# ccaven/tinyslam

Hardware: AMD Instinct MI355X
Metric: ORB extract throughput, 1280x720 (frames/sec; Mkeypoints/sec alongside) (higher is better)
Workload: dtype f32; 1 GPU; BASELINE.json configs[3]: batch of 256 independent 1280x720 RGBA frames per GPU, device-resident, full ORB (FAST-12 + orientation + blur + BRIEF-256); frames_per_gpu_per_batch=256, width=1280, height=720, hierarchy_depth=2, max_features=8192, content=default, mode=literal, input=rgba, pipeline=default, fp_contract=0, angle_bins=0, batches_in_flight=1, collate=none (1 GPU)

## Files before the change

### include/tinyorb.h

```cpp
#ifndef TINYORB_H
#define TINYORB_H

#include <stddef.h>
#include <stdint.h>

#ifdef __cplusplus
extern "C" {
#endif

#define TINYORB_ABI_VERSION 5

#define ORB_OK 0
#define ORB_EINVAL 1
#define ORB_EHIP 2
#define ORB_ECAPACITY 3
#define ORB_ESTATE 4

#define ORB_MAX_HIERARCHY_DEPTH 10

typedef struct OrbExtent3d {
    uint32_t width;
    uint32_t height;
    uint32_t depth_or_array_layers;
} OrbExtent3d;
// ... 260 lines not shown
#define ORB_TRACK_MATCHED 2u

typedef struct {
    uint32_t prev;
    uint32_t next;
    uint32_t head_index;
    uint16_t head_frame;
    uint16_t tail_frame;
} OrbTrack;

typedef struct {
    uint32_t keypoints;
    uint32_t links_in;
    uint32_t links_out;
    uint32_t keyframe;
    uint32_t ref_keyframe;
    uint32_t shared;
    uint32_t reserved[2];
} OrbTrackFrame;

int orb_track_consecutive(OrbProgram *p, uint32_t n_frames, const OrbTrackParams *params, void *stream);
int orb_track_read(OrbProgram *p, uint32_t frame, OrbTrack *dst, size_t n);
int orb_track_frames(OrbProgram *p, OrbTrackFrame *dst, size_t n);

void orb_corner_level0_xy(const CornerData *c, float *x0, float *y0);

#define ORB_PLANE_GRAY 0
#define ORB_PLANE_BLUR 1
int orb_debug_read_plane(OrbProgram *p, uint32_t frame, int kind, uint32_t level, uint16_t *dst, size_t n_texels);
int orb_level_size(const OrbProgram *p, uint32_t level, uint32_t *width, uint32_t *height);
int orb_debug_f32_to_f16(OrbProgram *p, const float *src, uint16_t *dst, size_t n);
int orb_debug_angle_code(OrbProgram *p, const float *cy, const float *cx, uint32_t *dst, size_t n);
int orb_debug_rot_table(OrbProgram *p, int16_t *dst, size_t n_entries, uint32_t *codes, uint32_t *pitch);
int orb_debug_pose_buffers(OrbProgram *p, void **matches, void **poses, void **points);

#define ORB_KERNEL_COUNT 25
int orb_profile_enable(OrbProgram *p, int enable);
int orb_profile_reset(OrbProgram *p);
int orb_profile_get(OrbProgram *p, int id, double *total_ms, uint64_t *launches);
const char *orb_kernel_name(int id);

#define ORB_SYN_GRADIENT 1u
#define ORB_SYN_BLOBS 2u
#define ORB_SYN_WEDGES 4u
#define ORB_SYN_NOISE 8u
#define ORB_SYN_Y8 16u
int orb_synth_frames_device(OrbProgram *p, uint8_t *frames_dev, uint32_t n_frames, uint32_t seed0, uint32_t flags,
                            uint8_t **out_dev);
int orb_debug_stamps(OrbProgram *p, unsigned long long *dst, size_t n);
int orb_copy_to_host(OrbProgram *p, void *dst_host, const void *src_dev, size_t nbytes);

#ifdef __cplusplus
}
#endif
#endif
```

### tinyslam_amd/csrc/orb_api.hip

```cpp
#include <hip/hip_runtime.h>
#include <chrono>
#include <cmath>

#include <cstdarg>
#include <cstdio>
#include <cstdlib>
#include <cstring>
#include <new>
#include <optional>
#include <string>
#include <algorithm>
#include <vector>

#include "../../include/tinyorb.h"
#include "orb_front_launch.h"
#include "orb_kernels_fused.h"
#include "orb_kernels_brief.h"
#include "orb_kernels_intended.h"
#include "orb_kernels_staged.h"
#include "orb_kernels_collate.h"
#include "orb_kernels_match.h"
#include "orb_kernels_verify.h"
#include "orb_kernels_epipolar.h"
#include "orb_kernels_guide.h"
// ... 155 lines not shown
        bool no_swizzle = false, quiet = false;
        bool front_generic = false, front_trace = false;
        int phase_mask = -1, brief_i_mask = -1, lds_pad = 0;
    } env;
    uint32_t* dv_count = nullptr;
    CornerData* dv_corners = nullptr;
    CornerDescriptor* dv_desc = nullptr;
    uint16_t* d_gray = nullptr;
    uint16_t* d_blur = nullptr;
    uint16_t* d_blur_rowc = nullptr;
    uint32_t blur_qa[kMaxLevels] = {0};
    uint32_t* d_counts = nullptr;
    CornerData* d_corners = nullptr;
    CornerDescriptor* d_desc = nullptr;
    uint32_t* out_counts[2] = {nullptr, nullptr};
    CornerData* out_corners[2] = {nullptr, nullptr};
    CornerDescriptor* out_desc[2] = {nullptr, nullptr};
    CornerData* d_seg = nullptr;
    uint32_t* d_seg_counts = nullptr;
    uint32_t* d_seg_before = nullptr;
    uint64_t* d_nf_mask[2] = {nullptr, nullptr};
    BandGeom bands{};
    RowsGeom rows{};
    BriefTGeom brieft{};
    bool use_brief_t = false;
    uint32_t band_rows_lvl[kMaxLevels] = {0};
    uint32_t ln_threads[kMaxLevels] = {0};
    uint32_t tile_w_lvl[kMaxLevels] = {0};
    uint32_t seg_classes = 1;
    uint32_t* d_pattern = nullptr;
    float* d_cos = nullptr;
    float* d_sin = nullptr;
    uint4* d_rot = nullptr;
    unsigned long long* d_stamps = nullptr;

    uint32_t* h_count = nullptr;
    uint32_t* d_single_done = nullptr;
    hipEvent_t single_done_ev = nullptr;
    uint32_t single_seq = 0;
    CornerData* h_corners = nullptr;
    CornerDescriptor* h_desc = nullptr;
    bool single_valid = false;

    uint32_t last_batch = 0;
    hipStream_t last_stream = nullptr;
    bool planes_valid = false;
    bool fused = false;
    uint32_t max_lds = 0;
    uint32_t n_cus = 256;

    bool profiling = false;
    std::vector<ProfSpan> pending;
    std::vector<hipEvent_t> event_pool;
    double prof_ms[ORB_KERNEL_COUNT] = {0};
    uint64_t prof_n[ORB_KERNEL_COUNT] = {0};

    std::string pipeline_note;
    std::string err;
};

namespace {

int fail(OrbProgram* p, int code, const char* fmt, ...) {
    char buf[512];
    va_list ap;
    va_start(ap, fmt);
// ... 367 lines not shown
    for (uint32_t m = 0; m < p->pyr.depth; m++) {
        g.flat_end[m] = rg.flat_end[m];
        g.qa[m] = rg.qa[m];
        g.row_base[m] = rows + (uint32_t)kBriefHalo;
        rows += p->pyr.h[m] + 2u * (uint32_t)kBriefHalo + 8u;
    }
    g.rows_padded = rows;
    g.oob = p->oob;
    *out = g;
    if (getenv("TINYORB_BRIEF_ROWS")) return false;
    return rg.n_slots >= 1u && rg.n_slots * n_classes <= kBriefTMaxSlots && rows <= kBriefTMaxRows;
}

int launch_brief(OrbProgram* p, hipStream_t s, uint32_t n, const RowsGeom& rows_geom, const uint16_t* d_blur,
                 const uint16_t* d_blur_rowc, const uint32_t* seg_counts, uint32_t* seg_before, const CornerData* seg,
                 uint32_t* d_counts, CornerData* d_corners, CornerDescriptor* d_desc, uint32_t f0 = 0) {
    const uint32_t cap = p->cfg.max_features;
    const BriefTables tab{p->d_pattern, p->d_cos, p->d_sin, p->d_rot};
    const bool use_t = p->use_brief_t;
    {
        LaunchScope ls(p, s, KID_PREFIX);
        hipLaunchKernelGGL(k_slot_prefix, dim3(n), dim3(64), 0, s, seg_counts, seg_before, d_counts, rows_geom.n_slots,
                           rows_geom.seg_cap, use_t ? p->brieft.n_classes : 1u);
    }
    if (use_t) {
        const BriefTGeom& tg = p->brieft;
        const dim3 grid(n, (cap + (uint32_t)kBriefNfChunk - 1u) / (uint32_t)kBriefNfChunk);
        const uint32_t mask_words = brief_mask_words(cap);
        uint64_t* const nf_mask = p->d_nf_mask[p->cur_set] + (size_t)f0 * mask_words;
        {
            LaunchScope ls(p, s, KID_BRIEF_T);
#define BRIEF_T_LAUNCH(ROT_)                                                                                                         \
    hipLaunchKernelGGL((k_brief_t<kBriefTWaves, ROT_>), dim3(n, (cap + kBriefTThreads - 1u) / kBriefTThreads), dim3(kBriefTThreads), \
                       brieft_lds_bytes(tg), s, d_blur_rowc, p->pyr, tg, seg_counts, seg_before, seg, d_corners, cap, d_desc, tab, nf_mask, mask_words)
            switch (rot_form(p->opt.fp_contract)) {
                case 1: BRIEF_T_LAUNCH(1); break;
                case 2: BRIEF_T_LAUNCH(2); break;
                default: BRIEF_T_LAUNCH(0); break;
            }
#undef BRIEF_T_LAUNCH
        }
        LaunchScope ls(p, s, KID_BRIEF_NF);
#define BRIEF_NF_LAUNCH(OOB_, TABLE_)                                                                                                  \
    hipLaunchKernelGGL((k_brief_nf<OOB_, TABLE_>), grid, dim3(256), 0, s, d_blur, d_blur_rowc, p->pyr, tg, d_corners, cap, d_desc, tab, \
                       nf_mask, mask_words)
        const bool table = p->pyr.depth > 2u;
        if (p->oob != kOobZero) {
            if (table) BRIEF_NF_LAUNCH(true, true); else BRIEF_NF_LAUNCH(true, false);
        } else {
            if (table) BRIEF_NF_LAUNCH(false, true); else BRIEF_NF_LAUNCH(false, false);
        }
#undef BRIEF_NF_LAUNCH
    } else {
        LaunchScope ls(p, s, KID_BRIEF_ROWS);
        RowsGeom rg = rows_geom;
        rg.oob = p->oob;
        rg.fp = p->opt.fp_contract;
        rg.split = 1u;
        while (rg.split < 16u && rg.n_slots * n * rg.split < 2048u) rg.split *= 2u;
        hipLaunchKernelGGL(k_brief_rows, dim3(rg.n_slots * rg.split, n), dim3(256), 0, s, d_blur, d_blur_rowc, p->pyr, rg,
                           seg_counts, seg_before, seg, d_corners, cap, d_desc, tab);
    }
    return ORB_OK;
}

FrontGeom fused_level_geometry(const OrbProgram* p, uint32_t lvl, uint32_t gw, uint32_t gh, uint32_t n) {
    const Pyramid& pyr = p->pyr;
// ... 662 lines not shown
        for (uint32_t m = 0; m < p->pyr.depth; m++) {
            const uint32_t gw = ((width + 7u) / 8u) * 8u, gh = ((height + 7u) / 8u) * 8u;
            p->score_layout.off[m] = off;
            p->score_layout.pitch[m] = gw + 2u;
            off += (gw + 2u) * (gh + 2u);
            width /= 2u;
            height /= 2u;
        }
        p->score_layout.stride = (off + 63u) & ~63u;
        p->cap_prov = (uint32_t)std::min<uint64_t>(std::max<uint64_t>(p->pyr.stride, cap), 1u << 24);
        if (p->opt.flags & ORB_FLAG_NMS)
        CREATE_TRY(hipMalloc(&p->d_score_planes, B * (size_t)p->score_layout.stride * sizeof(float)));
        CREATE_TRY(hipMalloc(&p->d_prov_counts, B * sizeof(uint32_t)));
        CREATE_TRY(hipMalloc(&p->d_prov, B * (size_t)p->cap_prov * sizeof(CornerData)));
        CREATE_TRY(hipMalloc(&p->d_prov_scores, B * (size_t)p->cap_prov * sizeof(float)));
        if (p->intended && (p->opt.flags & ORB_FLAG_NMS)) {
            CREATE_TRY(hipMalloc(&p->d_prov2_counts, B * sizeof(uint32_t)));
            CREATE_TRY(hipMalloc(&p->d_prov2, B * (size_t)p->cap_prov * sizeof(CornerData)));
            CREATE_TRY(hipMalloc(&p->d_prov2_scores, B * (size_t)p->cap_prov * sizeof(float)));
        }
    }
    CREATE_TRY(hipMalloc(&p->d_pattern, 256 * sizeof(uint32_t)));
    CREATE_TRY(hipMalloc(&p->d_cos, ORB_ANGLE_STEPS_FULL * sizeof(float)));
    CREATE_TRY(hipMalloc(&p->d_sin, ORB_ANGLE_STEPS_FULL * sizeof(float)));
    CREATE_TRY(hipMemcpy(p->d_pattern, ORB_BRIEF_PATTERN, 1024, hipMemcpyHostToDevice));
    CREATE_TRY(hipMemcpy(p->d_cos, ORB_COS_BITS, ORB_ANGLE_STEPS_FULL * 4, hipMemcpyHostToDevice));
    CREATE_TRY(hipMemcpy(p->d_sin, ORB_SIN_BITS, ORB_ANGLE_STEPS_FULL * 4, hipMemcpyHostToDevice));
    {
        const uint32_t n_codes = p->fused_i ? (p->opt.angle_bins ? p->opt.angle_bins : (uint32_t)ORB_ANGLE_STEPS_FULL) : (uint32_t)ORB_ANGLE_STEPS;
        const int pitch = p->fused_i ? (int)p->itiles.pitch : kNfPatchCols;
        CREATE_TRY(hipMalloc(&p->d_rot, (size_t)n_codes * 64u * sizeof(uint4)));
        hipLaunchKernelGGL(k_rot_table, dim3(n_codes), dim3(64), 0, p->stream, p->d_pattern, p->d_cos, p->d_sin, pitch, p->fused_i ? 1 : 0, p->d_rot,
                           p->opt.fp_contract, p->fused_i ? p->opt.angle_bins : 0u);
        CREATE_TRY(hipGetLastError());
        CREATE_TRY(hipStreamSynchronize(p->stream));
    }
    if (p->fused && getenv("TINYORB_STAMPS")) {
        CREATE_TRY(hipMalloc(&p->d_stamps, 32 * sizeof(unsigned long long)));
        CREATE_TRY(hipMemset(p->d_stamps, 0, 32 * sizeof(unsigned long long)));
    }
    CREATE_TRY(hipHostMalloc(&p->h_count, kSingleCountWords * sizeof(uint32_t), hipHostMallocDefault));
    memset(p->h_count, 0, kSingleCountWords * sizeof(uint32_t));
    CREATE_TRY(hipMalloc(&p->d_single_done, sizeof(uint32_t)));
    CREATE_TRY(hipMemset(p->d_single_done, 0, sizeof(uint32_t)));
    CREATE_TRY(hipHostMalloc(&p->h_corners, cap * sizeof(CornerData), hipHostMallocDefault));
    CREATE_TRY(hipHostMalloc(&p->h_desc, cap * sizeof(CornerDescriptor), hipHostMallocDefault));
    {
        void *dc = nullptr, *dk = nullptr, *dd = nullptr;
        if (hipHostGetDevicePointer(&dc, p->h_count, 0) == hipSuccess && hipHostGetDevicePointer(&dk, p->h_corners, 0) == hipSuccess &&
            hipHostGetDevicePointer(&dd, p->h_desc, 0) == hipSuccess) {
            p->dv_count = static_cast<uint32_t*>(dc);
            p->dv_corners = static_cast<CornerData*>(dk);
            p->dv_desc = static_cast<CornerDescriptor*>(dd);
        } else {
            (void)hipGetLastError();
        }
    }
#undef CREATE_TRY
    *out = p;
    return ORB_OK;
}

void orb_program_destroy(OrbProgram* p) {
    if (!p) return;
    (void)hipSetDevice(p->device);
    if (p->stream) (void)hipStreamSynchronize(p->stream);
// ... 5 lines not shown
    (void)hipFree(p->d_input);
    (void)hipFree(p->d_input_alt);
    for (hipEvent_t ev : p->in_uploaded)
        if (ev) (void)hipEventDestroy(ev);
    (void)hipFree(p->d_gray);
    (void)hipFree(p->d_blur);
    (void)hipFree(p->d_blur_rowc);
    for (int set = 0; set < 2; set++) {
        (void)hipFree(p->out_counts[set]);
        (void)hipFree(p->out_corners[set]);
        (void)hipFree(p->out_desc[set]);
    }
    (void)hipFree(p->d_seg);
    (void)hipFree(p->d_seg_counts);
    (void)hipFree(p->d_seg_before);
    for (int set = 0; set < 2; set++) (void)hipFree(p->d_nf_mask[set]);
    (void)hipFree(p->d_score_planes);
    (void)hipFree(p->d_prov_counts);
    (void)hipFree(p->d_prov);
    (void)hipFree(p->d_prov_scores);
    (void)hipFree(p->d_xband_counts);
    (void)hipFree(p->d_iseg);
    (void)hipFree(p->d_iseg_scores);
    (void)hipFree(p->d_iseg_counts);
    (void)hipFree(p->d_iseg_before);
    (void)hipFree(p->d_thr_key);
    (void)hipFree(p->d_prov2_counts);
    (void)hipFree(p->d_prov2);
    (void)hipFree(p->d_prov2_scores);
    (void)hipFree(p->d_pattern);
    (void)hipFree(p->d_cos);
    (void)hipFree(p->d_sin);
    if (p->d_rot) (void)hipFree(p->d_rot);
    (void)hipFree(p->d_stamps);
    for (int st = 0; st < ST_COUNT; st++) {
        free_stage_buffers(p, st);
        if (p->stage[st].done) (void)hipEventDestroy(p->stage[st].done);
    }
    if (p->single_done_ev) (void)hipEventDestroy(p->single_done_ev);
    if (p->h_count) (void)hipHostFree(p->h_count);
    if (p->d_single_done) (void)hipFree(p->d_single_done);
    if (p->h_corners) (void)hipHostFree(p->h_corners);
    if (p->h_desc) (void)hipHostFree(p->h_desc);
    if (p->stream) (void)hipStreamDestroy(p->stream);
    if (p->copy_stream) (void)hipStreamDestroy(p->copy_stream);
    if (p->order_event) (void)hipEventDestroy(p->order_event);
    for (hipEvent_t ev : p->upload_events) (void)hipEventDestroy(ev);
    if (p->upload_done) (void)hipEventDestroy(p->upload_done);
    for (int set = 0; set < 2; set++) {
        (void)hipFree(p->d_pack_c[set]);
        (void)hipFree(p->d_pack_d[set]);
        if (p->h_pack_counts[set]) (void)hipHostFree(p->h_pack_counts[set]);
        if (p->h_pack_offsets[set]) (void)hipHostFree(p->h_pack_offsets[set]);
        if (p->pack_event[set]) (void)hipEventDestroy(p->pack_event[set]);
    }
    delete p;
}

static int pick_input_slab(OrbProgram* p, bool ahead, uint32_t* slab_out, uint8_t** dst, bool* appended) {
    if (ahead && p->in_pending >= 2u)
        return fail(p, ORB_ESTATE, "two images are already waiting for extract_corners");
    if (int rc = ensure_input(p)) return rc;
    uint32_t slab;
    if (p->in_pending == 0u || ahead) {
        slab = p->in_pending == 0u ? p->in_last : (p->in_queue[0] ^ 1u);
        *appended = true;
// ... 1204 lines not shown
    HIP_TRY(p, hipSetDevice(p->device));
    float *d_cy = nullptr, *d_cx = nullptr;
    uint32_t* d_dst = nullptr;
    HIP_TRY(p, hipMalloc(&d_cy, n * sizeof(float)));
    hipError_t e = hipMalloc(&d_cx, n * sizeof(float));
    if (e == hipSuccess) e = hipMalloc(&d_dst, n * sizeof(uint32_t));
    if (e == hipSuccess) e = hipMemcpy(d_cy, cy, n * sizeof(float), hipMemcpyHostToDevice);
    if (e == hipSuccess) e = hipMemcpy(d_cx, cx, n * sizeof(float), hipMemcpyHostToDevice);
    if (e == hipSuccess) {
        hipLaunchKernelGGL(k_probe_angle, dim3((unsigned)((n + 255) / 256)), dim3(256), 0, p->stream, d_cy, d_cx, d_dst, n);
        e = hipStreamSynchronize(p->stream);
    }
    if (e == hipSuccess) e = hipMemcpy(dst, d_dst, n * sizeof(uint32_t), hipMemcpyDeviceToHost);
    (void)hipFree(d_cy);
    (void)hipFree(d_cx);
    (void)hipFree(d_dst);
    if (e != hipSuccess) return fail(p, ORB_EHIP, "debug_angle_code: %s", hipGetErrorString(e));
    return ORB_OK;
}

int orb_debug_rot_table(OrbProgram* p, int16_t* dst, size_t n_entries, uint32_t* codes, uint32_t* pitch) {
    if (!p) return ORB_EINVAL;
    if (!p->d_rot) return fail(p, ORB_ESTATE, "this program has no rotated-pattern table");
    const uint32_t n_codes = p->fused_i ? (p->opt.angle_bins ? p->opt.angle_bins : (uint32_t)ORB_ANGLE_STEPS_FULL) : (uint32_t)ORB_ANGLE_STEPS;
    if (codes) *codes = n_codes;
    if (pitch) *pitch = p->fused_i ? p->itiles.pitch : (uint32_t)kNfPatchCols;
    const size_t n = std::min(n_entries, (size_t)n_codes * 512u);
    if (n && !dst) return fail(p, ORB_EINVAL, "dst is NULL");
    HIP_TRY(p, hipSetDevice(p->device));
    if (n) HIP_TRY(p, hipMemcpy(dst, p->d_rot, n * sizeof(int16_t), hipMemcpyDeviceToHost));
    return ORB_OK;
}

int orb_profile_enable(OrbProgram* p, int enable) {
    if (!p) return ORB_EINVAL;
    p->profiling = enable != 0;
    return ORB_OK;
}

int orb_profile_reset(OrbProgram* p) {
    if (!p) return ORB_EINVAL;
    HIP_TRY(p, hipSetDevice(p->device));
    if (int rc = drain_profile(p)) return rc;
    for (int i = 0; i < ORB_KERNEL_COUNT; i++) {
        p->prof_ms[i] = 0;
        p->prof_n[i] = 0;
    }
    return ORB_OK;
}

int orb_profile_get(OrbProgram* p, int id, double* total_ms, uint64_t* launches) {
    if (!p || id < 0 || id >= ORB_KERNEL_COUNT) return ORB_EINVAL;
    HIP_TRY(p, hipSetDevice(p->device));
    if (int rc = drain_profile(p)) return rc;
    if (total_ms) *total_ms = p->prof_ms[id];
    if (launches) *launches = p->prof_n[id];
    return ORB_OK;
}

int orb_synth_frames_device(OrbProgram* p, uint8_t* frames_dev, uint32_t n_frames, uint32_t seed0, uint32_t flags,
                            uint8_t** out_dev) {
    if (!p) return ORB_EINVAL;
    if (n_frames == 0) return fail(p, ORB_EINVAL, "n_frames is 0");
    HIP_TRY(p, hipSetDevice(p->device));
    if (!frames_dev) {
        if (n_frames > p->max_batch) return fail(p, ORB_EINVAL, "n_frames %u > max_batch %u", n_frames, p->max_batch);
// ... 39 lines not shown
```

### tinyslam_amd/csrc/orb_kernels_brief.h

```cpp
#pragma once
#include "orb_kernels_fused.h"

namespace orb {

constexpr int kBriefTThreads = 256;
constexpr int kBriefTWaves = 6;
constexpr uint32_t kBriefTMaxSlots = 8192;
constexpr uint32_t kBriefTMaxRows = 12288;
__host__ __device__ inline uint32_t brief_mask_words(uint32_t cap) { return 4u * ((cap + (uint32_t)kBriefTThreads - 1u) / (uint32_t)kBriefTThreads); }

struct BriefTGeom {
    uint32_t n_slots, seg_cap;
    uint32_t n_classes;
    uint32_t flat_end[kMaxLevels];
    uint32_t qa[kMaxLevels];
    uint32_t row_base[kMaxLevels];
    uint32_t rows_padded;
    uint32_t oob;
};

__host__ __device__ inline uint32_t brieft_lds_bytes(const BriefTGeom& g) {
    return (g.n_slots * g.n_classes + 1u) * 4u + ((g.rows_padded + 1u) & ~1u) * 2u;
}

__device__ __forceinline__ constexpr int pat_ax(int j) { return ORB_BRIEF_PATTERN[4 * j + 0]; }
__device__ __forceinline__ constexpr int pat_ay(int j) { return ORB_BRIEF_PATTERN[4 * j + 1]; }
__device__ __forceinline__ constexpr int pat_bx(int j) { return ORB_BRIEF_PATTERN[4 * j + 2]; }
__device__ __forceinline__ constexpr int pat_by(int j) { return ORB_BRIEF_PATTERN[4 * j + 3]; }

__device__ __forceinline__ uint32_t wave_inclusive_sum(uint32_t x) {
    int v = (int)x;
    v += __builtin_amdgcn_update_dpp(0, v, 0x111, 0xf, 0xf, true);
    v += __builtin_amdgcn_update_dpp(0, v, 0x112, 0xf, 0xf, true);
    v += __builtin_amdgcn_update_dpp(0, v, 0x114, 0xf, 0xf, true);
    v += __builtin_amdgcn_update_dpp(0, v, 0x118, 0xf, 0xf, true);
    v += __builtin_amdgcn_update_dpp(0, v, 0x142, 0xa, 0xf, true);
    v += __builtin_amdgcn_update_dpp(0, v, 0x143, 0xc, 0xf, true);
    return (uint32_t)v;
}

__device__ __forceinline__ void store_host_u32(uint32_t* p, uint32_t v) { *p = v; }
__device__ __forceinline__ void store_host_16(void* p, uint4 v) { *reinterpret_cast<uint4*>(p) = v; }

__device__ __forceinline__ uint32_t push_gt(uint32_t word, uint32_t a, uint32_t b) {
    return __builtin_amdgcn_alignbit(word, b - a, 31);
}

__device__ __forceinline__ void brief_t_stage_rows(uint16_t* rows, const uint16_t* __restrict__ src, const Pyramid& pyr,
                                                   const BriefTGeom& bg, uint32_t tid, uint32_t n_threads = kBriefTThreads) {
    uint32_t m = 0;
    for (uint32_t i = tid; i < bg.rows_padded; i += n_threads) {
        while (m + 1u < pyr.depth && i + (uint32_t)kBriefHalo >= bg.row_base[m + 1u]) m++;
        const uint32_t y = i - bg.row_base[m];
        uint16_t v = 0;
        if (y < pyr.h[m]) v = src[pyr.row_off[m] + y];
        else if (bg.oob != kOobZero) v = src[pyr.row_off[m] + (uint32_t)oob_index((int)y, (int)pyr.h[m], bg.oob)];
        rows[i] = v;
    }
}

template <int CHUNK = kBriefTThreads, bool STAGED = false, int ROT = 0, bool MASK = false>
__device__ __forceinline__ void brief_t_body(uint8_t* lds_raw, uint32_t frame, uint32_t chunk, const uint16_t* __restrict__ blur_rowc,
                                             const Pyramid& pyr, const BriefTGeom& bg, const uint32_t* __restrict__ seg_counts,
                                             const uint32_t* __restrict__ seg_before, const CornerData* __restrict__ segments,
                                             CornerData* __restrict__ corners, uint32_t cap,
                                             CornerDescriptor* __restrict__ descriptors, const BriefTables& tab,
                                             CornerData* __restrict__ host_corners = nullptr,
                                             CornerDescriptor* __restrict__ host_descriptors = nullptr,
                                             uint64_t* __restrict__ nf_mask = nullptr, uint32_t mask_words = 0) {
    static_assert(!MASK || (CHUNK == kBriefTThreads && !STAGED), "the mask is the batch kernel's: 256 keypoints, four words");
    const uint32_t n_ent = bg.n_slots * bg.n_classes;
    uint32_t* const before = reinterpret_cast<uint32_t*>(lds_raw);
    uint16_t* const rows = reinterpret_cast<uint16_t*>(before + n_ent + 1u);
    __shared__ uint32_t lv[kMaxLevels][2];

    const uint32_t tid = threadIdx.x;
    const size_t sbase = (size_t)frame * n_ent;
    uint32_t stored_total;
    if (STAGED) {
        if (tid < pyr.depth) lv[tid][0] = bg.flat_end[tid], lv[tid][1] = bg.row_base[tid];
        __syncthreads();
        stored_total = before[n_ent];
    } else {
        stored_total = seg_before[sbase + n_ent - 1u] + min(seg_counts[sbase + n_ent - 1u], bg.seg_cap);
    }
    const uint32_t n_frame = min(stored_total, cap);
    const uint32_t k0 = chunk * (uint32_t)CHUNK;
    uint64_t* const mask_word = MASK ? nf_mask + (size_t)frame * mask_words + (k0 >> 6) + (tid >> 6) : nullptr;
    if (k0 >= n_frame) {
        if (MASK && (tid & 63u) == 0u) *mask_word = 0ull;
        return;
    }

    if (!STAGED) {
        for (uint32_t s = tid; s < n_ent; s += kBriefTThreads) before[s] = seg_before[sbase + s];
        if (tid == 0) before[n_ent] = stored_total;
        if (tid < pyr.depth) lv[tid][0] = bg.flat_end[tid], lv[tid][1] = bg.row_base[tid];
        brief_t_stage_rows(rows, blur_rowc + (size_t)frame * pyr.row_stride, pyr, bg, tid);
        __syncthreads();
    }

    const uint32_t k = k0 + tid;
    const bool live = k < n_frame;
    if (!MASK && (tid >= (uint32_t)CHUNK || !live)) return;
    uint4 fetched = make_uint4(0u, 0u, 0u, 0u);
    if (!MASK || live) {
        uint32_t lo = 0, hi = n_ent;
        while (hi - lo > 1u) {
            const uint32_t mid = (lo + hi) >> 1;
            if (before[mid] <= k)
                lo = mid;
            else
                hi = mid;
        }
        const uint32_t cls = lo >= bg.n_slots ? 1u : 0u, slot = lo - cls * bg.n_slots;
        fetched = *reinterpret_cast<const uint4*>(
            &segments[(((size_t)frame * bg.n_slots + slot) * bg.n_classes + cls) * bg.seg_cap + (k - before[lo])]);
        *reinterpret_cast<uint4*>(&corners[(size_t)frame * cap + k]) = fetched;
        if (host_corners) store_host_16(&host_corners[k], fetched);
    }
    const uint4 rec = fetched;
    const uint32_t lvl = min(rec.w, pyr.depth - 1u);
    if constexpr (MASK) {
        const bool flat = live && rec.x >= (uint32_t)kBriefHalo && rec.x < lv[lvl][0];
        const uint64_t not_flat = __ballot(live && !flat);
        if ((tid & 63u) == 0u) *mask_word = not_flat;
        if (!flat) return;
    } else {
        if (!(rec.x >= (uint32_t)kBriefHalo && rec.x < lv[lvl][0])) return;
    }

    uint32_t d[8];
    uint4* const o = reinterpret_cast<uint4*>(descriptors + (size_t)frame * cap + k);
    if (bg.n_classes == 2u && k0 + (tid & ~63u) + 64u <= before[bg.n_slots]) {
        const uint16_t* base0 = rows + lv[lvl][1] + rec.y - kBriefHalo;
#pragma unroll
        for (int wd = 0; wd < 8; wd++) {
            uint32_t acc = 0;
#pragma unroll
            for (int i = 31; i >= 0; i--) {
                const int j = wd * 32 + i;
                acc = push_gt(acc, base0[pat_ay(j) + kBriefHalo], base0[pat_by(j) + kBriefHalo]);
            }
            d[wd] = acc;
        }
        o[0] = make_uint4(d[0], d[1], d[2], d[3]);
        o[1] = make_uint4(d[4], d[5], d[6], d[7]);
        if (host_descriptors) {
            store_host_16(reinterpret_cast<uint4*>(host_descriptors + k), make_uint4(d[0], d[1], d[2], d[3]));
            store_host_16(reinterpret_cast<uint4*>(host_descriptors + k) + 1, make_uint4(d[4], d[5], d[6], d[7]));
        }
        return;
    }
    const uint32_t code = min(rec.z, (uint32_t)(ORB_ANGLE_STEPS - 1));
    const float ct = tab.cos_tab[code], st = tab.sin_tab[code], nst = -st;
    const uint16_t* base = rows + lv[lvl][1] + rec.y;
#pragma unroll
    for (int wd = 0; wd < 8; wd++) {
        float ctw = ct, nstw = nst;
        asm volatile("" : "+v"(ctw), "+v"(nstw));
        uint32_t acc = 0;
#pragma unroll
        for (int i = 31; i >= 0; i--) {
            const int j = wd * 32 + i;
            float ray, rby;
            if constexpr (ROT == 1) {
                const float a2 = nstw * (float)pat_ax(j), b2 = nstw * (float)pat_bx(j);
                ray = __builtin_fmaf(ctw, (float)pat_ay(j), a2), rby = __builtin_fmaf(ctw, (float)pat_by(j), b2);
            } else if constexpr (ROT == 2) {
                const float a3 = ctw * (float)pat_ay(j), b3 = ctw * (float)pat_by(j);
                ray = __builtin_fmaf(nstw, (float)pat_ax(j), a3), rby = __builtin_fmaf(nstw, (float)pat_bx(j), b3);
            } else {
                const float a2 = nstw * (float)pat_ax(j), a3 = ctw * (float)pat_ay(j);
                const float b2 = nstw * (float)pat_bx(j), b3 = ctw * (float)pat_by(j);
                ray = a2 + a3, rby = b2 + b3;
            }
            acc = push_gt(acc, base[(int)ray], base[(int)rby]);
        }
        d[wd] = acc;
    }
    o[0] = make_uint4(d[0], d[1], d[2], d[3]);
    o[1] = make_uint4(d[4], d[5], d[6], d[7]);
    if (host_descriptors) {
        store_host_16(reinterpret_cast<uint4*>(host_descriptors + k), make_uint4(d[0], d[1], d[2], d[3]));
        store_host_16(reinterpret_cast<uint4*>(host_descriptors + k) + 1, make_uint4(d[4], d[5], d[6], d[7]));
    }
}

template <int kWavesPerSimd, int ROT = 0>
__global__ __launch_bounds__(kBriefTThreads, kWavesPerSimd) void k_brief_t(const uint16_t* __restrict__ blur_rowc, Pyramid pyr, BriefTGeom bg,
                                                                const uint32_t* __restrict__ seg_counts,
                                                                const uint32_t* __restrict__ seg_before,
                                                                const CornerData* __restrict__ segments,
                                                                CornerData* __restrict__ corners, uint32_t cap,
                                                                CornerDescriptor* __restrict__ descriptors, BriefTables tab,
                                                                uint64_t* __restrict__ nf_mask, uint32_t mask_words) {
    extern __shared__ __attribute__((aligned(16))) uint8_t lds_raw[];
    brief_t_body<kBriefTThreads, false, ROT, true>(lds_raw, blockIdx.x, blockIdx.y, blur_rowc, pyr, bg, seg_counts, seg_before, segments, corners, cap, descriptors, tab,
                                                   nullptr, nullptr, nf_mask, mask_words);
}

constexpr int kNfPatchCols = 48, kNfPatchRows = 2 * kBriefHalo + 1;
constexpr int kNfPatchHalfs = kNfPatchRows * kNfPatchCols;

__global__ __launch_bounds__(64) void k_rot_table(const uint32_t* __restrict__ pattern, const float* __restrict__ cos_tab,
                                                  const float* __restrict__ sin_tab, int pitch, int intended, uint4* __restrict__ out,
                                                  uint32_t fp = 0u, uint32_t angle_bins = 0u) {
    const uint32_t code = angle_bins ? (blockIdx.x * 6284u + 3142u) / angle_bins : blockIdx.x, lane = threadIdx.x;
    const float ct = cos_tab[code], st = sin_tab[code], nst = -st;
    uint32_t w[4];
#pragma unroll
    for (int e = 0; e < 4; e++) {
        const uint32_t pk = pattern[64u * (uint32_t)e + lane];
        const float pax = (float)(int8_t)(pk & 255u), pay = (float)(int8_t)((pk >> 8) & 255u);
        const float pbx = (float)(int8_t)((pk >> 16) & 255u), pby = (float)(int8_t)(pk >> 24);
        float rax, ray, rbx, rby;
        if (intended) {
            const float a0 = ct * pax, a1 = nst * pay, a2 = st * pax, a3 = ct * pay;
            const float b0 = ct * pbx, b1 = nst * pby, b2 = st * pbx, b3 = ct * pby;
            rax = a0 + a1, ray = a2 + a3, rbx = b0 + b1, rby = b2 + b3;
        } else {
            rotate_fp(ct, st, nst, pax, pay, rot_form(fp), &rax, &ray);
            rotate_fp(ct, st, nst, pbx, pby, rot_form(fp), &rbx, &rby);
        }
        const int oa = 2 * ((int)ray * pitch + (int)rax), ob = 2 * ((int)rby * pitch + (int)rbx);
        w[e] = ((uint32_t)oa & 0xffffu) | ((uint32_t)ob << 16);
    }
    out[(size_t)blockIdx.x * 64u + lane] = make_uint4(w[0], w[1], w[2], w[3]);
}
__device__ __forceinline__ int rot_a(uint32_t w) { return (int)(int16_t)(w & 0xffffu); }
__device__ __forceinline__ int rot_b(uint32_t w) { return (int)w >> 16; }

// ... 207 lines not shown
```

### tinyslam_amd/orb.py

```python
import ctypes
import importlib.util
import os
from dataclasses import dataclass, field

import numpy as np

_PKG = os.path.dirname(os.path.abspath(__file__))
LIB_PATH = os.environ.get("TINYORB_LIB") or os.path.join(os.path.dirname(os.path.abspath(__file__)), "libtinyorb.so")

ORB_OK, ORB_EINVAL, ORB_EHIP, ORB_ECAPACITY, ORB_ESTATE = 0, 1, 2, 3, 4
ORB_PLANE_GRAY, ORB_PLANE_BLUR = 0, 1
ORB_KERNEL_COUNT = 25
ORB_FLAG_STAGED = 1
ORB_FLAG_DOUBLE_OUTPUT = 2
ORB_FLAG_NMS = 4
ORB_FLAG_INTENDED = 8
ORB_FLAG_INPUT_Y8 = 16
ORB_FLAG_SINGLE_BLOCKING_WAIT = 32
ORB_OOB_ZERO, ORB_OOB_CLAMP, ORB_OOB_UMIN = 0, 1, 2
OOB_POLICIES = {"zero": ORB_OOB_ZERO, "clamp": ORB_OOB_CLAMP, "umin": ORB_OOB_UMIN}
ORB_FP_CONTRACT_LUMINANCE, ORB_FP_CONTRACT_BLUR, ORB_FP_CONTRACT_ROTATION, ORB_FP_CONTRACT_ALL, ORB_FP_LAST_TERM_FIRST = 1, 2, 4, 7, 8
TRANSPORT_RECORD_WORDS = 10
SYN_GRADIENT, SYN_BLOBS, SYN_WEDGES, SYN_NOISE = 1, 2, 4, 8
SYN_ALL = 15

CORNER_DTYPE = np.dtype([("x", "<u4"), ("y", "<u4"), ("angle", "<u4"), ("octave", "<u4")])
MATCH_DTYPE = np.dtype([("index", "<u4"), ("distance", "<u2"), ("second", "<u2")])
ORB_MATCH_NONE = 0xFFFFFFFF
DESCRIPTOR_DTYPE = np.dtype([("bits", "u1", (32,))])
VERIFY_MODEL_DTYPE = np.dtype([("h", "<f4", (9,)), ("candidates", "<u4"), ("inliers", "<u4"), ("hypothesis", "<u4"),
                               ("status", "<u4"), ("reserved", "<u4", (3,))])
ORB_VERIFY_OK, ORB_VERIFY_FEW, ORB_VERIFY_DEGENERATE, ORB_VERIFY_MINIMAL = 0, 1, 2, 3
ORB_VERIFY_MAX_HYPOTHESES = 4096
ORB_GUIDE_VERIFIED, ORB_GUIDE_IDENTITY, ORB_GUIDE_HOST = 0, 1, 2
ORB_GUIDE_SCALE_RADIUS = 1
ORB_BAND_VERIFIED, ORB_BAND_HOST = 0, 1
ORB_BAND_SCALE = 1
POSE_DTYPE = np.dtype([("r", "<f4", (9,)), ("t", "<f4", (3,)), ("inliers", "<u4"), ("good", "<u4"), ("second", "<u4"), ("status", "<u4")])
POINT_DTYPE = np.dtype([("x", "<f4"), ("y", "<f4"), ("z", "<f4"), ("flags", "<u4")])
ORB_POSE_OK, ORB_POSE_NOMODEL, ORB_POSE_FEW, ORB_POSE_AMBIGUOUS, ORB_POSE_LOW_PARALLAX = 0, 1, 2, 3, 4
ORB_POINT_GOOD, ORB_POINT_PARALLAX = 1, 2
FRAME_POSE_DTYPE = np.dtype([("r", "<f4", (9,)), ("t", "<f4", (3,)), ("scale", "<f4"), ("step", "<f4"), ("origin", "<u4"),
                             ("shared", "<u4"), ("consistent", "<u4"), ("status", "<u4"), ("reserved", "<u4", (2,))])
ORB_TRAJ_CHAINED, ORB_TRAJ_START, ORB_TRAJ_RESTART_FEW, ORB_TRAJ_RESTART_SPREAD, ORB_TRAJ_LOST, ORB_TRAJ_ORIGIN = 0, 1, 2, 3, 4, 5
ORB_TRAJ_NEED_PARALLAX = 1
ORB_TRACK_VERIFIED, ORB_TRACK_GUIDED, ORB_TRACK_MATCHED = 0, 1, 2
TRACK_DTYPE = np.dtype([("prev", "<u4"), ("next", "<u4"), ("head_index", "<u4"), ("head_frame", "<u2"), ("tail_frame", "<u2")])
TRACK_FRAME_DTYPE = np.dtype([("keypoints", "<u4"), ("links_in", "<u4"), ("links_out", "<u4"), ("keyframe", "<u4"),
                              ("ref_keyframe", "<u4"), ("shared", "<u4"), ("reserved", "<u4", (2,))])

EXPORTS = [
    "orb_abi_version", "orb_pipeline", "orb_last_error", "orb_kernel_name", "orb_program_create", "orb_program_destroy",
    "orb_write_input_image", "orb_set_threshold", "orb_extract_corners", "orb_read_corners",
    "orb_read_descriptors", "orb_extract_batch_device", "orb_extract_batch_host", "orb_batch_sync",
    "orb_batch_counts", "orb_batch_read", "orb_batch_select_output", "orb_batch_device_buffers", "orb_level_size",
    "orb_debug_read_plane", "orb_debug_f32_to_f16", "orb_debug_angle_code", "orb_debug_rot_table", "orb_profile_enable",
    "orb_profile_reset", "orb_profile_get", "orb_synth_frames_device", "orb_copy_to_host", "orb_debug_stamps",
    "orb_match_consecutive", "orb_match_read", "orb_corner_level0_xy",
    "orb_batch_read_all", "orb_batch_compact_device", "orb_host_alloc", "orb_host_free", "orb_stream_sync",
    "orb_program_stream", "orb_pipeline_note", "orb_batch_pack", "orb_batch_fetch",
    "orb_batch_pack_transport", "orb_unpack_transport",
    "orb_node_create", "orb_node_destroy", "orb_node_last_error", "orb_node_device_count", "orb_node_program",
    "orb_node_shard", "orb_node_extract_batch", "orb_node_extract_batch_host", "orb_node_collate",
    "orb_node_read_collated", "orb_node_collate_begin", "orb_node_collate_end", "orb_node_pending",
    "orb_extract_batch_pinned", "orb_upload_sync", "orb_node_exchange_backend", "orb_node_rccl_pairs",
    "orb_write_input_image_pinned", "orb_node_set_results", "orb_node_shard_result",
    "orb_verify_consecutive", "orb_verify_read", "orb_match_guided", "orb_match_guided_read",
    "orb_track_consecutive", "orb_track_read", "orb_track_frames", "orb_verify_epipolar", "orb_verify_epipolar_read",
    "orb_match_epipolar", "orb_match_epipolar_read", "orb_pose_consecutive", "orb_pose_read",
    "orb_trajectory_consecutive", "orb_trajectory_read", "orb_debug_pose_buffers",
]


def level0_xy(corners):
    s = np.left_shift(1, corners["octave"].astype(np.int64)).astype(np.float32)
    return ((corners["x"].astype(np.float32) + np.float32(0.5)) * s - np.float32(0.5),
            (corners["y"].astype(np.float32) + np.float32(0.5)) * s - np.float32(0.5))


class OrbError(RuntimeError):
    def __init__(self, code, msg):
        super().__init__("tinyorb error %d: %s" % (code, msg))
        self.code = code


class _Extent3d(ctypes.Structure):
    _fields_ = [("width", ctypes.c_uint32), ("height", ctypes.c_uint32), ("depth_or_array_layers", ctypes.c_uint32)]


# ... 72 lines not shown
    L = ctypes.CDLL(path)
    vp, u32, sz = ctypes.c_void_p, ctypes.c_uint32, ctypes.c_size_t
    L.orb_abi_version.restype = u32
    L.orb_last_error.restype = ctypes.c_char_p
    L.orb_last_error.argtypes = [vp]
    L.orb_kernel_name.restype = ctypes.c_char_p
    L.orb_pipeline.restype = ctypes.c_char_p
    L.orb_pipeline.argtypes = [vp]
    L.orb_pipeline_note.restype = ctypes.c_char_p
    L.orb_pipeline_note.argtypes = [vp]
    L.orb_kernel_name.argtypes = [ctypes.c_int]
    L.orb_program_create.argtypes = [ctypes.POINTER(_Config), ctypes.POINTER(_Options), ctypes.POINTER(vp)]
    L.orb_program_destroy.argtypes = [vp]
    L.orb_program_destroy.restype = None
    L.orb_write_input_image.argtypes = [vp, vp, sz]
    L.orb_write_input_image_pinned.argtypes = [vp, vp, sz]
    L.orb_set_threshold.argtypes = [vp, ctypes.c_float]
    L.orb_extract_corners.argtypes = [vp, ctypes.POINTER(u32)]
    L.orb_read_corners.argtypes = [vp, vp, sz]
    L.orb_read_descriptors.argtypes = [vp, vp, sz]
    L.orb_extract_batch_device.argtypes = [vp, vp, u32, vp]
    L.orb_extract_batch_host.argtypes = [vp, vp, u32]
    L.orb_batch_sync.argtypes = [vp]
    L.orb_batch_counts.argtypes = [vp, vp, u32]
    L.orb_batch_read.argtypes = [vp, u32, vp, vp, sz]
    L.orb_batch_select_output.argtypes = [vp, u32]
    L.orb_batch_device_buffers.argtypes = [vp, ctypes.POINTER(vp), ctypes.POINTER(vp), ctypes.POINTER(vp)]
    L.orb_level_size.argtypes = [vp, u32, ctypes.POINTER(u32), ctypes.POINTER(u32)]
    L.orb_debug_pose_buffers.argtypes = [vp, ctypes.POINTER(vp), ctypes.POINTER(vp), ctypes.POINTER(vp)]
    L.orb_debug_read_plane.argtypes = [vp, u32, ctypes.c_int, u32, vp, sz]
    L.orb_debug_f32_to_f16.argtypes = [vp, vp, vp, sz]
    L.orb_debug_angle_code.argtypes = [vp, vp, vp, vp, sz]
    L.orb_debug_rot_table.argtypes = [vp, vp, sz, vp, vp]
    L.orb_match_consecutive.argtypes = [vp, u32, vp]
    L.orb_match_read.argtypes = [vp, u32, vp, ctypes.c_size_t]
    L.orb_verify_consecutive.argtypes = [vp, u32, ctypes.POINTER(_VerifyParams), vp]
    L.orb_verify_read.argtypes = [vp, u32, vp, vp, sz]
    L.orb_verify_epipolar.argtypes = [vp, u32, ctypes.POINTER(_VerifyParams), vp]
    L.orb_verify_epipolar_read.argtypes = [vp, u32, vp, vp, sz]
    L.orb_match_guided.argtypes = [vp, u32, ctypes.POINTER(_GuideParams), vp, vp]
    L.orb_match_guided_read.argtypes = [vp, u32, vp, sz]
    L.orb_match_epipolar.argtypes = [vp, u32, ctypes.POINTER(_BandParams), vp, vp]
    L.orb_match_epipolar_read.argtypes = [vp, u32, vp, sz]
    L.orb_pose_consecutive.argtypes = [vp, u32, ctypes.POINTER(_PoseParams), vp]
    L.orb_pose_read.argtypes = [vp, u32, vp, vp, sz]
    L.orb_trajectory_consecutive.argtypes = [vp, u32, ctypes.POINTER(_TrajectoryParams), vp]
    L.orb_trajectory_read.argtypes = [vp, u32, vp, vp, sz]
    L.orb_track_consecutive.argtypes = [vp, u32, ctypes.POINTER(_TrackParams), vp]
    L.orb_track_read.argtypes = [vp, u32, vp, sz]
    L.orb_track_frames.argtypes = [vp, vp, sz]
    L.orb_profile_enable.argtypes = [vp, ctypes.c_int]
    L.orb_profile_reset.argtypes = [vp]
    L.orb_profile_get.argtypes = [vp, ctypes.c_int, ctypes.POINTER(ctypes.c_double), ctypes.POINTER(ctypes.c_uint64)]
    L.orb_synth_frames_device.argtypes = [vp, vp, u32, u32, u32, ctypes.POINTER(vp)]
    L.orb_copy_to_host.argtypes = [vp, vp, vp, sz]
    L.orb_debug_stamps.argtypes = [vp, vp, sz]
    L.orb_corner_level0_xy.argtypes = [vp, ctypes.POINTER(ctypes.c_float), ctypes.POINTER(ctypes.c_float)]
    L.orb_corner_level0_xy.restype = None
    L.orb_batch_read_all.argtypes = [vp, u32, vp, vp, vp, vp, sz, vp]
    L.orb_batch_compact_device.argtypes = [vp, u32, vp, vp, vp, vp, sz, vp]
    L.orb_batch_pack.argtypes = [vp, u32, vp]
    L.orb_batch_fetch.argtypes = [vp, u32, vp, vp, vp, vp, sz, vp]
    L.orb_batch_pack_transport.argtypes = [vp, u32, u32, vp, sz, vp, vp]
    L.orb_unpack_transport.argtypes = [vp, vp, u32, vp, vp, vp, vp, vp, vp]
    L.orb_host_alloc.argtypes = [sz, ctypes.POINTER(vp)]
    L.orb_host_free.argtypes = [vp]
# ... 391 lines not shown
        return self._lib.orb_pipeline_note(self._handle()).decode()

    def level_size(self, level):
        w, h = ctypes.c_uint32(), ctypes.c_uint32()
        self._check(self._lib.orb_level_size(self._handle(), level, ctypes.byref(w), ctypes.byref(h)))
        return w.value, h.value

    def read_plane(self, kind, level, frame=0):
        w, h = self.level_size(level)
        out = np.zeros((h, w), dtype=np.uint16)
        self._check(self._lib.orb_debug_read_plane(self._handle(), frame, kind, level, _ptr(out), out.size))
        return out

    def device_f32_to_f16(self, src):
        src = np.ascontiguousarray(src, dtype=np.float32)
        out = np.zeros(src.shape, dtype=np.uint16)
        self._check(self._lib.orb_debug_f32_to_f16(self._handle(), _ptr(src), _ptr(out), src.size))
        return out

    def device_angle_code(self, cy, cx):
        cy = np.ascontiguousarray(cy, dtype=np.float32)
        cx = np.ascontiguousarray(cx, dtype=np.float32)
        out = np.zeros(cy.shape, dtype=np.uint32)
        self._check(self._lib.orb_debug_angle_code(self._handle(), _ptr(cy), _ptr(cx), _ptr(out), cy.size))
        return out

    def rot_table(self):
        codes, pitch = ctypes.c_uint32(0), ctypes.c_uint32(0)
        self._check(self._lib.orb_debug_rot_table(self._handle(), None, 0, ctypes.byref(codes), ctypes.byref(pitch)))
        out = np.zeros((codes.value, 64, 4, 2), dtype=np.int16)
        self._check(self._lib.orb_debug_rot_table(self._handle(), _ptr(out), out.size, None, None))
        return out, pitch.value

    def profile_enable(self, on=True):
        self._check(self._lib.orb_profile_enable(self._handle(), 1 if on else 0))

    def profile_reset(self):
        self._check(self._lib.orb_profile_reset(self._handle()))

    def profile(self):
        out = {}
        for i in range(ORB_KERNEL_COUNT):
            ms, n = ctypes.c_double(), ctypes.c_uint64()
            self._check(self._lib.orb_profile_get(self._handle(), i, ctypes.byref(ms), ctypes.byref(n)))
            if n.value:
                out[self._lib.orb_kernel_name(i).decode()] = (ms.value, n.value)
        return out

    def synth_frames_device(self, n_frames, seed0, flags=SYN_ALL, frames_dev_ptr=None):
        out = ctypes.c_void_p()
        self._check(self._lib.orb_synth_frames_device(self._handle(), ctypes.c_void_p(frames_dev_ptr) if frames_dev_ptr else None,
                                                      n_frames, seed0 & 0xFFFFFFFF, flags, ctypes.byref(out)))
        return out.value

    def debug_stamps(self, n_workgroups):
        out = np.zeros((n_workgroups, 6), dtype=np.uint64)
        self._check(self._lib.orb_debug_stamps(self._handle(), _ptr(out), out.size))
        return out

    def copy_to_host(self, dev_ptr, nbytes):
        out = np.zeros(nbytes, dtype=np.uint8)
        self._check(self._lib.orb_copy_to_host(self._handle(), _ptr(out), ctypes.c_void_p(dev_ptr), nbytes))
        return out


class OrbNode:
# ... 100 lines not shown
```

Baseline: 551,500 frames/s.

## Use precomputed rotated sample-row table for BRIEF in non-uniform class waves

Adds a per-angle table of rotated BRIEF sample offsets, packed as row-scaled byte pairs and built once at program creation. In the batch BRIEF-T kernel, waves that are not fully in the uniform two-class case now compact their flat keypoints and compute descriptors cooperatively. Eight lanes share one keypoint and read the packed offsets instead of doing per-bit float rotation. The mask path also forces the aligned row-base branch. This trades float math for table loads and a wave-level compaction step through LDS, adding a small new buffer and a debug readback API.

```diff
diff --git a/include/tinyorb.h b/include/tinyorb.h
--- a/include/tinyorb.h
+++ b/include/tinyorb.h
@@ -316,6 +316,7 @@
 int orb_debug_f32_to_f16(OrbProgram *p, const float *src, uint16_t *dst, size_t n);
 int orb_debug_angle_code(OrbProgram *p, const float *cy, const float *cx, uint32_t *dst, size_t n);
 int orb_debug_rot_table(OrbProgram *p, int16_t *dst, size_t n_entries, uint32_t *codes, uint32_t *pitch);
+int orb_debug_rot_rows(OrbProgram *p, int8_t *dst, size_t n_entries, uint32_t *codes);
 int orb_debug_pose_buffers(OrbProgram *p, void **matches, void **poses, void **points);
 
 #define ORB_KERNEL_COUNT 25
diff --git a/tinyslam_amd/csrc/orb_api.hip b/tinyslam_amd/csrc/orb_api.hip
--- a/tinyslam_amd/csrc/orb_api.hip
+++ b/tinyslam_amd/csrc/orb_api.hip
@@ -211,6 +211,7 @@
     float* d_cos = nullptr;
     float* d_sin = nullptr;
     uint4* d_rot = nullptr;
+    uint2* d_rot_rows = nullptr;
     unsigned long long* d_stamps = nullptr;
 
     uint32_t* h_count = nullptr;
@@ -644,7 +645,8 @@
             LaunchScope ls(p, s, KID_BRIEF_T);
 #define BRIEF_T_LAUNCH(ROT_)                                                                                                         \
     hipLaunchKernelGGL((k_brief_t<kBriefTWaves, ROT_>), dim3(n, (cap + kBriefTThreads - 1u) / kBriefTThreads), dim3(kBriefTThreads), \
-                       brieft_lds_bytes(tg), s, d_blur_rowc, p->pyr, tg, seg_counts, seg_before, seg, d_corners, cap, d_desc, tab, nf_mask, mask_words)
+                       brieft_lds_bytes(tg), s, d_blur_rowc, p->pyr, tg, seg_counts, seg_before, seg, d_corners, cap, d_desc, tab, nf_mask, mask_words, \
+                       p->d_rot_rows)
             switch (rot_form(p->opt.fp_contract)) {
                 case 1: BRIEF_T_LAUNCH(1); break;
                 case 2: BRIEF_T_LAUNCH(2); break;
@@ -1373,6 +1375,11 @@
         CREATE_TRY(hipMalloc(&p->d_rot, (size_t)n_codes * 64u * sizeof(uint4)));
         hipLaunchKernelGGL(k_rot_table, dim3(n_codes), dim3(64), 0, p->stream, p->d_pattern, p->d_cos, p->d_sin, pitch, p->fused_i ? 1 : 0, p->d_rot,
                            p->opt.fp_contract, p->fused_i ? p->opt.angle_bins : 0u);
+        if (p->use_brief_t) {
+            CREATE_TRY(hipMalloc(&p->d_rot_rows, (size_t)ORB_ANGLE_STEPS * 64u * sizeof(uint2)));
+            hipLaunchKernelGGL(k_rot_rows, dim3(ORB_ANGLE_STEPS), dim3(64), 0, p->stream, p->d_pattern, p->d_cos, p->d_sin,
+                               rot_form(p->opt.fp_contract), p->d_rot_rows);
+        }
         CREATE_TRY(hipGetLastError());
         CREATE_TRY(hipStreamSynchronize(p->stream));
     }
@@ -1444,6 +1451,7 @@
     (void)hipFree(p->d_cos);
     (void)hipFree(p->d_sin);
     if (p->d_rot) (void)hipFree(p->d_rot);
+    (void)hipFree(p->d_rot_rows);
     (void)hipFree(p->d_stamps);
     for (int st = 0; st < ST_COUNT; st++) {
         free_stage_buffers(p, st);
@@ -2714,6 +2722,17 @@
     return ORB_OK;
 }
 
+int orb_debug_rot_rows(OrbProgram* p, int8_t* dst, size_t n_entries, uint32_t* codes) {
+    if (!p) return ORB_EINVAL;
+    if (!p->d_rot_rows) return fail(p, ORB_ESTATE, "this program has no sample-row table");
+    if (codes) *codes = (uint32_t)ORB_ANGLE_STEPS;
+    const size_t n = std::min(n_entries, (size_t)ORB_ANGLE_STEPS * 512u);
+    if (n && !dst) return fail(p, ORB_EINVAL, "dst is NULL");
+    HIP_TRY(p, hipSetDevice(p->device));
+    if (n) HIP_TRY(p, hipMemcpy(dst, p->d_rot_rows, n, hipMemcpyDeviceToHost));
+    return ORB_OK;
+}
+
 int orb_profile_enable(OrbProgram* p, int enable) {
     if (!p) return ORB_EINVAL;
     p->profiling = enable != 0;
diff --git a/tinyslam_amd/csrc/orb_kernels_brief.h b/tinyslam_amd/csrc/orb_kernels_brief.h
--- a/tinyslam_amd/csrc/orb_kernels_brief.h
+++ b/tinyslam_amd/csrc/orb_kernels_brief.h
@@ -44,6 +44,90 @@
 
 __device__ __forceinline__ uint32_t push_gt(uint32_t word, uint32_t a, uint32_t b) {
     return __builtin_amdgcn_alignbit(word, b - a, 31);
+}
+
+template <int ROT>
+__device__ __forceinline__ void rot_rows_ab(float ctw, float nstw, float ax, float ay, float bx, float by, float* ray_out, float* rby_out) {
+    float ray, rby;
+    if constexpr (ROT == 1) {
+        const float a2 = nstw * ax, b2 = nstw * bx;
+        ray = __builtin_fmaf(ctw, ay, a2), rby = __builtin_fmaf(ctw, by, b2);
+    } else if constexpr (ROT == 2) {
+        const float a3 = ctw * ay, b3 = ctw * by;
+        ray = __builtin_fmaf(nstw, ax, a3), rby = __builtin_fmaf(nstw, bx, b3);
+    } else {
+        const float a2 = nstw * ax, a3 = ctw * ay;
+        const float b2 = nstw * bx, b3 = ctw * by;
+        ray = a2 + a3, rby = b2 + b3;
+    }
+    *ray_out = ray, *rby_out = rby;
+}
+
+__global__ __launch_bounds__(64) void k_rot_rows(const uint32_t* __restrict__ pattern, const float* __restrict__ cos_tab,
+                                                 const float* __restrict__ sin_tab, int form, uint2* __restrict__ out) {
+    const uint32_t code = blockIdx.x, lane = threadIdx.x;
+    const float ct = cos_tab[code], st = sin_tab[code], nst = -st;
+    uint32_t w[2] = {0u, 0u};
+#pragma unroll
+    for (int e = 0; e < 4; e++) {
+        const uint32_t pk = pattern[64u * (uint32_t)e + lane];
+        const float pax = (float)(int8_t)(pk & 255u), pay = (float)(int8_t)((pk >> 8) & 255u);
+        const float pbx = (float)(int8_t)((pk >> 16) & 255u), pby = (float)(int8_t)(pk >> 24);
+        float ray, rby;
+        if (form == 1) rot_rows_ab<1>(ct, nst, pax, pay, pbx, pby, &ray, &rby);
+        else if (form == 2) rot_rows_ab<2>(ct, nst, pax, pay, pbx, pby, &ray, &rby);
+        else rot_rows_ab<0>(ct, nst, pax, pay, pbx, pby, &ray, &rby);
+        const uint32_t pair = ((uint32_t)(2 * (int)ray) & 255u) | (((uint32_t)(2 * (int)rby) & 255u) << 8);
+        w[e >> 1] |= pair << (16 * (e & 1));
+    }
+    out[(size_t)code * 64u + lane] = make_uint2(w[0], w[1]);
+}
+
+__device__ __forceinline__ void brief_t_table_rows(bool flat, const uint16_t* rows, uint32_t row_index, uint32_t code,
+                                                   const uint2* __restrict__ rot_rows, CornerDescriptor* desc_wave) {
+    static_assert(kBriefTMaxRows <= (1u << 14) && ORB_ANGLE_STEPS <= (1 << 12), "row index, angle code and lane share one word");
+    __shared__ uint32_t packed[kBriefTThreads / 64][64];
+    const uint32_t lane = threadIdx.x & 63u, wave = threadIdx.x >> 6;
+    const uint64_t m = __ballot(flat);
+    const uint32_t n = (uint32_t)__builtin_popcountll(m);
+    if (n == 0u) return;
+    const uint32_t rank = __builtin_amdgcn_mbcnt_hi((uint32_t)(m >> 32), __builtin_amdgcn_mbcnt_lo((uint32_t)m, 0u));
+    if (flat) packed[wave][rank] = row_index | (code << 14) | (lane << 26);
+    __builtin_amdgcn_fence(__ATOMIC_RELEASE, "wavefront");
+    __builtin_amdgcn_wave_barrier();
+    const uint32_t q = lane & 7u, sub = lane >> 3;
+    uint32_t pkn;
+    uint4 tn[4];
+    auto fetch = [&](uint32_t r0) {
+        pkn = packed[wave][min(r0 + sub, n - 1u)];
+        const uint4* const t = reinterpret_cast<const uint4*>(rot_rows + (((pkn >> 14) & 0xfffu) * 64u + 8u * q));
+#pragma unroll
+        for (int i = 0; i < 4; i++) tn[i] = t[i];
+    };
+    fetch(0u);
+    for (uint32_t r0 = 0; r0 < n; r0 += 8u) {
+        const uint32_t pk = pkn;
+        const uint32_t w[8] = {tn[0].x, tn[0].y, tn[0].z, tn[0].w, tn[1].x, tn[1].y, tn[1].z, tn[1].w};
+        const uint32_t w2[8] = {tn[2].x, tn[2].y, tn[2].z, tn[2].w, tn[3].x, tn[3].y, tn[3].z, tn[3].w};
+        if (r0 + 8u < n) fetch(r0 + 8u);
+        const char* const own = reinterpret_cast<const char*>(rows + (pk & 0x3fffu));
+        uint32_t acc[4] = {0u, 0u, 0u, 0u};
+#pragma unroll
+        for (int i = 7; i >= 0; i--) {
+#pragma unroll
+            for (int e = 0; e < 4; e++) {
+                const uint32_t word = i < 4 ? w[2 * i + (e >> 1)] : w2[2 * (i - 4) + (e >> 1)];
+                const uint32_t pair = word >> (16 * (e & 1));
+                const int oa = (int)(int8_t)(pair & 255u), ob = (int)(int8_t)((pair >> 8) & 255u);
+                acc[e] = push_gt(acc[e], *reinterpret_cast<const uint16_t*>(own + oa), *reinterpret_cast<const uint16_t*>(own + ob));
+            }
+        }
+        if (r0 + sub < n) {
+            uint8_t* const out = reinterpret_cast<uint8_t*>(desc_wave + (pk >> 26)) + 4u * (q >> 2) + (q & 3u);
+#pragma unroll
+            for (int e = 0; e < 4; e++) out[8 * e] = (uint8_t)acc[e];
+        }
+    }
 }
 
 __device__ __forceinline__ void brief_t_stage_rows(uint16_t* rows, const uint16_t* __restrict__ src, const Pyramid& pyr,
@@ -67,7 +151,8 @@
                                              CornerDescriptor* __restrict__ descriptors, const BriefTables& tab,
                                              CornerData* __restrict__ host_corners = nullptr,
                                              CornerDescriptor* __restrict__ host_descriptors = nullptr,
-                                             uint64_t* __restrict__ nf_mask = nullptr, uint32_t mask_words = 0) {
+                                             uint64_t* __restrict__ nf_mask = nullptr, uint32_t mask_words = 0,
+                                             const uint2* __restrict__ rot_rows = nullptr) {
     static_assert(!MASK || (CHUNK == kBriefTThreads && !STAGED), "the mask is the batch kernel's: 256 keypoints, four words");
     const uint32_t n_ent = bg.n_slots * bg.n_classes;
     uint32_t* const before = reinterpret_cast<uint32_t*>(lds_raw);
@@ -125,6 +210,11 @@
         const bool flat = live && rec.x >= (uint32_t)kBriefHalo && rec.x < lv[lvl][0];
         const uint64_t not_flat = __ballot(live && !flat);
         if ((tid & 63u) == 0u) *mask_word = not_flat;
+        if (!(bg.n_classes == 2u && k0 + (tid & ~63u) + 64u <= before[bg.n_slots])) {
+            brief_t_table_rows(flat, rows, lv[lvl][1] + rec.y, min(rec.z, (uint32_t)(ORB_ANGLE_STEPS - 1)), rot_rows,
+                               descriptors + (size_t)frame * cap + k0 + (tid & ~63u));
+            return;
+        }
         if (!flat) return;
     } else {
         if (!(rec.x >= (uint32_t)kBriefHalo && rec.x < lv[lvl][0])) return;
@@ -132,7 +222,7 @@
 
     uint32_t d[8];
     uint4* const o = reinterpret_cast<uint4*>(descriptors + (size_t)frame * cap + k);
-    if (bg.n_classes == 2u && k0 + (tid & ~63u) + 64u <= before[bg.n_slots]) {
+    if (MASK || (bg.n_classes == 2u && k0 + (tid & ~63u) + 64u <= before[bg.n_slots])) {
         const uint16_t* base0 = rows + lv[lvl][1] + rec.y - kBriefHalo;
 #pragma unroll
         for (int wd = 0; wd < 8; wd++) {
@@ -164,17 +254,7 @@
         for (int i = 31; i >= 0; i--) {
             const int j = wd * 32 + i;
             float ray, rby;
-            if constexpr (ROT == 1) {
-                const float a2 = nstw * (float)pat_ax(j), b2 = nstw * (float)pat_bx(j);
-                ray = __builtin_fmaf(ctw, (float)pat_ay(j), a2), rby = __builtin_fmaf(ctw, (float)pat_by(j), b2);
-            } else if constexpr (ROT == 2) {
-                const float a3 = ctw * (float)pat_ay(j), b3 = ctw * (float)pat_by(j);
-                ray = __builtin_fmaf(nstw, (float)pat_ax(j), a3), rby = __builtin_fmaf(nstw, (float)pat_bx(j), b3);
-            } else {
-                const float a2 = nstw * (float)pat_ax(j), a3 = ctw * (float)pat_ay(j);
-                const float b2 = nstw * (float)pat_bx(j), b3 = ctw * (float)pat_by(j);
-                ray = a2 + a3, rby = b2 + b3;
-            }
+            rot_rows_ab<ROT>(ctw, nstw, (float)pat_ax(j), (float)pat_ay(j), (float)pat_bx(j), (float)pat_by(j), &ray, &rby);
             acc = push_gt(acc, base[(int)ray], base[(int)rby]);
         }
         d[wd] = acc;
@@ -194,10 +274,11 @@
                                                                 const CornerData* __restrict__ segments,
                                                                 CornerData* __restrict__ corners, uint32_t cap,
                                                                 CornerDescriptor* __restrict__ descriptors, BriefTables tab,
-                                                                uint64_t* __restrict__ nf_mask, uint32_t mask_words) {
+                                                                uint64_t* __restrict__ nf_mask, uint32_t mask_words,
+                                                                const uint2* __restrict__ rot_rows) {
     extern __shared__ __attribute__((aligned(16))) uint8_t lds_raw[];
     brief_t_body<kBriefTThreads, false, ROT, true>(lds_raw, blockIdx.x, blockIdx.y, blur_rowc, pyr, bg, seg_counts, seg_before, segments, corners, cap, descriptors, tab,
-                                                   nullptr, nullptr, nf_mask, mask_words);
+                                                   nullptr, nullptr, nf_mask, mask_words, rot_rows);
 }
 
 constexpr int kNfPatchCols = 48, kNfPatchRows = 2 * kBriefHalo + 1;
diff --git a/tinyslam_amd/orb.py b/tinyslam_amd/orb.py
--- a/tinyslam_amd/orb.py
+++ b/tinyslam_amd/orb.py
@@ -54,7 +54,7 @@
     "orb_write_input_image", "orb_set_threshold", "orb_extract_corners", "orb_read_corners",
     "orb_read_descriptors", "orb_extract_batch_device", "orb_extract_batch_host", "orb_batch_sync",
     "orb_batch_counts", "orb_batch_read", "orb_batch_select_output", "orb_batch_device_buffers", "orb_level_size",
-    "orb_debug_read_plane", "orb_debug_f32_to_f16", "orb_debug_angle_code", "orb_debug_rot_table", "orb_profile_enable",
+    "orb_debug_read_plane", "orb_debug_f32_to_f16", "orb_debug_angle_code", "orb_debug_rot_table", "orb_debug_rot_rows", "orb_profile_enable",
     "orb_profile_reset", "orb_profile_get", "orb_synth_frames_device", "orb_copy_to_host", "orb_debug_stamps",
     "orb_match_consecutive", "orb_match_read", "orb_corner_level0_xy",
     "orb_batch_read_all", "orb_batch_compact_device", "orb_host_alloc", "orb_host_free", "orb_stream_sync",
@@ -193,6 +193,8 @@
     L.orb_debug_f32_to_f16.argtypes = [vp, vp, vp, sz]
     L.orb_debug_angle_code.argtypes = [vp, vp, vp, vp, sz]
     L.orb_debug_rot_table.argtypes = [vp, vp, sz, vp, vp]
+    if hasattr(L, "orb_debug_rot_rows"):
+        L.orb_debug_rot_rows.argtypes = [vp, vp, sz, vp]
     L.orb_match_consecutive.argtypes = [vp, u32, vp]
     L.orb_match_read.argtypes = [vp, u32, vp, ctypes.c_size_t]
     L.orb_verify_consecutive.argtypes = [vp, u32, ctypes.POINTER(_VerifyParams), vp]
@@ -650,6 +652,13 @@
         self._check(self._lib.orb_debug_rot_table(self._handle(), _ptr(out), out.size, None, None))
         return out, pitch.value
 
+    def rot_rows(self):
+        codes = ctypes.c_uint32(0)
+        self._check(self._lib.orb_debug_rot_rows(self._handle(), None, 0, ctypes.byref(codes)))
+        out = np.zeros((codes.value, 64, 4, 2), dtype=np.int8)
+        self._check(self._lib.orb_debug_rot_rows(self._handle(), _ptr(out), out.size, None))
+        return out
+
     def profile_enable(self, on=True):
         self._check(self._lib.orb_profile_enable(self._handle(), 1 if on else 0))
 
```

New measurement: 555,100 frames/s, median of 6. No clear change (+0.7%).
